# liyheng/MAGPO

Measured on NVIDIA B200. Metric: end_to_end_training_agent_env_steps_per_sec, higher is better.
Workload: dtype f32

## Files before the change

### magpo_b200/csrc/gemm_tc.cu

```cuda
#include <cuda.h>

#include <stdlib.h>

#include <vector>

#include "common.cuh"
#include "kernels.cuh"
#include "tc_ptx.cuh"

namespace magpo {
namespace {

using tcp::TC_BM;
constexpr int TC_KC = 32;
constexpr int TC_CHUNK_BYTES = TC_BM * TC_KC * 4;
constexpr int TC_CONV_THREADS = 256;
constexpr int TC_THREADS = 256 + TC_CONV_THREADS;
constexpr int TC_MAX_STAGES = 6;
constexpr uint32_t TC_SMEM_LIMIT = 227 * 1024;

struct TcParams {
  int M, N, K, BN, kchunks, stages, flags, num_row_tiles, tmem_cols, stacked ;
  const float* bias;
};
// ... 347 lines not shown
              CUtensorMapSwizzle swz = CU_TENSOR_MAP_SWIZZLE_128B) {
  EncodeTiledFn enc = get_encode();
  if (!enc) return false;
  cuuint64_t gdim[2] = {(cuuint64_t)cols, (cuuint64_t)rows};
  cuuint64_t gstride[1] = {(cuuint64_t)ld * 4};
  cuuint32_t box[2] = {(cuuint32_t)TC_KC, (cuuint32_t)box_rows};
  cuuint32_t estr[2] = {1, 1};
  return enc(tm, CU_TENSOR_MAP_DATA_TYPE_FLOAT32, 2, const_cast<float*>(ptr), gdim, gstride, box, estr, CU_TENSOR_MAP_INTERLEAVE_NONE,
             swz, CU_TENSOR_MAP_L2_PROMOTION_L2_128B, CU_TENSOR_MAP_FLOAT_OOB_FILL_NONE) == CUDA_SUCCESS;
}

bool env_tc_default() {
  const char* e = getenv("MAGPO_TENSOR_CORES");
  return !(e && e[0] == '0');
}
bool g_tc_enabled = env_tc_default();

}

bool tc_make_map(void* tensor_map, const float* ptr, int64_t rows, int cols, int ld, int box_rows) {
  return make_map(static_cast<CUtensorMap*>(tensor_map), ptr, rows, cols, ld, box_rows);
}
bool tc_make_map3(void* tensor_map, const float* ptr, int64_t T, int64_t rows, int cols, int box_rows) {
  EncodeTiledFn enc = get_encode();
  if (!enc) return false;
  cuuint64_t gdim[3] = {(cuuint64_t)cols, (cuuint64_t)rows, (cuuint64_t)T};
  cuuint64_t gstride[2] = {(cuuint64_t)cols * 4, (cuuint64_t)rows * cols * 4};
  cuuint32_t box[3] = {(cuuint32_t)TC_KC, (cuuint32_t)box_rows, 1};
  cuuint32_t estr[3] = {1, 1, 1};
  return enc(static_cast<CUtensorMap*>(tensor_map), CU_TENSOR_MAP_DATA_TYPE_FLOAT32, 3, const_cast<float*>(ptr), gdim, gstride, box, estr,
             CU_TENSOR_MAP_INTERLEAVE_NONE, CU_TENSOR_MAP_SWIZZLE_128B, CU_TENSOR_MAP_L2_PROMOTION_L2_128B,
             CU_TENSOR_MAP_FLOAT_OOB_FILL_NONE) == CUDA_SUCCESS;
}
void tc_set_enabled(bool on) { g_tc_enabled = on; }
bool tc_enabled() { return g_tc_enabled; }

int tc_prepare_region(cudaStream_t s, const float* base, int64_t n, float* hi, float* lo) {
  if (n <= 0) return MAGPO_OK;
  split_region_kernel<<<(unsigned)std::min<int64_t>(ceil_div(n, 256), 4 * kNumSMs), 256, 0, s>>>(n, base, hi, lo);
  MAGPO_LAUNCH_OK();
  auto overlaps = [](const float* a, int64_t na, const float* b, int64_t nb) { return a < b + nb && b < a + na; };
  std::vector<TcRegion>& g_regions = ctx().regions;
  for (size_t i = 0; i < g_regions.size();) {
    const TcRegion& r = g_regions[i];
    if (overlaps(r.base, r.n, base, n) || overlaps(r.base, r.n, hi, n) || overlaps(r.base, r.n, lo, n) ||
        overlaps(r.hi, r.n, base, n) || overlaps(r.lo, r.n, base, n))
      g_regions.erase(g_regions.begin() + (long)i);
    else
      ++i;
  }
  g_regions.push_back(TcRegion{base, n, hi, lo});
  return MAGPO_OK;
}

bool tc_lookup(const float* w, const float** hi, const float** lo) {
  const std::vector<TcRegion>& g_regions = ctx().regions;
  for (auto it = g_regions.rbegin(); it != g_regions.rend(); ++it) {
    const TcRegion& r = *it;
    if (w >= r.base && w < r.base + r.n) {
      *hi = r.hi + (w - r.base);
      *lo = r.lo + (w - r.base);
      return true;
    }
  }
  return false;
}
// ... 146 lines not shown
```

### magpo_b200/csrc/kernels.cuh

```cuda
#pragma once
#include "common.cuh"

namespace magpo {

constexpr int kD = 64;
constexpr int kH = 128;
constexpr int kMaxActions = 32;
constexpr int kMaxAgents = 8;

enum { GEMM_ACCUMULATE = 1, GEMM_RELU = 2 };

struct Wref {
  const float* w;
  int ldw;
  const float* wt;
  int ldwt;
};
inline Wref wref(const float* w, int ldw, const float* wt = nullptr, int ldwt = 0) { return Wref{w, ldw, wt, ldwt}; }

int gemm_nn(cudaStream_t s, int64_t M, int N, int K, const float* X, int ldx, Wref W, const float* bias, float* Y,
            int ldy, int flags);
void tc_set_enabled(bool on);
bool tc_enabled();
int tc_prepare_region(cudaStream_t s, const float* base, int64_t n, float* hi, float* lo);
bool tc_lookup(const float* w, const float** hi, const float** lo);
bool tc_supported(int64_t M, int N, int K, const float* X, int ldx, const float* Y, int ldy, int ldb);
int gemm_tc(cudaStream_t s, int64_t M, int N, int K, const float* X, int ldx, const float* Bhi, const float* Blo, int ldb,
            const float* bias, float* Y, int ldy, int flags);
bool tc_tn_supported(int64_t M, int N, int K, const float* X, int ldx, const float* dY, int ldy, const float* dW, int ldw);
int gemm_tc_tn(cudaStream_t s, int64_t M, int N, int K, const float* X, int ldx, const float* dY, int ldy, float* dW, int ldw);
bool tc_make_map(void* tensor_map, const float* ptr, int64_t rows, int cols, int ld, int box_rows);
bool tc_make_map3(void* tensor_map, const float* ptr, int64_t T, int64_t rows, int cols, int box_rows);
int gemm_tn(cudaStream_t s, int64_t M, int N, int K, const float* X, int ldx, const float* dY, int ldy, float* dW,
            int ldw);
void chain_set_enabled(bool on);
bool chain_supported(int64_t R);
int chain_gate_fwd(cudaStream_t s, int64_t R, const float* g, int ldg, const float* ret, const float* res, const float* gn_s,
                   const float* gn_b, const float* ln_s, const float* pe, const int32_t* step, int max_step, const float* W1T,
                   const float* W2T, const float* WpT, float* gated, float* o, float* y, float* ype, float* gl, float* hmid, float* proj,
                   int ldproj);
int chain_front_fwd(cudaStream_t s, int64_t R, int d, const float* obs, const float* obs_scale, const float* Wobs, int A, int a,
                    const int32_t* action, const float* Wa, const float* ln_s, const float* pe, const int32_t* step, int max_step,
                    const float* WqT, float* z0, float* x, float* xpe, float* qkvg);
int chain_tail_fwd(cudaStream_t s, int64_t R, const float* hmid, const float* res, const float* ln_s, const float* pe,
                   const int32_t* step, int max_step, const float* W1T, const float* WqT, int ldwq, const float* WhT, const float* h_bias,
                   const float* h2_s, const float* W3, const float* b3, int nout, float* f, float* x, float* xpe, float* q, int ldq,
                   float* zh, float* out);
int gru_scan_fwd(cudaStream_t s, int T, int N, int A, const float* gi, const float* WhT_hi, const float* WhT_lo, const float* bhn,
                 const uint8_t* done, float* rzn, float* ghn, float* Y, float* HU);
int gru_scan_bwd(cudaStream_t s, int T, int N, int A, const float* dY, const float* rzn, const float* ghn, const float* HU,
                 const uint8_t* done, const float* Wh_hi, const float* Wh_lo, float* dgi, float* dgh, float* dbi ,
                 float* dbhn );
int colsum(cudaStream_t s, int64_t M, int N, const float* dY, int ldy, float* db);
int transpose(cudaStream_t s, int R, int Cc, const float* in, float* out);

bool thin_k_ok(int K, int N, int ldw, const float* W, const float* Y, int ldy);
bool thin_n_ok(int K, int N, const float* X, int ldx);
bool obs_embed_ok(int d);
int thin_k_fwd(cudaStream_t s, int64_t R, int K, int N, const float* X, int ldx, const float* W, int ldw, const float* bias,
               float* Y, int ldy, int relu);
int thin_k_bwd(cudaStream_t s, int64_t R, int K, int N, const float* X, int ldx, const float* dY, int lddy, const float* relu_out,
               float* dW, int lddw, float* db);
int thin_n_fwd(cudaStream_t s, int64_t R, int K, int N, const float* X, int ldx, const float* W, int ldw, const float* bias,
               float* Y, int ldy);
int thin_n_bwd(cudaStream_t s, int64_t R, int K, int N, const float* X, int ldx, const float* dY, int lddy, const float* W, int ldw,
// ... 44 lines not shown
```

### magpo_b200/csrc/retention_chunk.cu

```cuda
#include "common.cuh"
#include "kernels.cuh"

namespace magpo {
namespace {

constexpr int RC_ROWS = 32;
constexpr int LDA = 68;
constexpr int LDB = 72;
constexpr int LDP = 36;
constexpr int LDPT = 40;

struct Frag {
  uint32_t h[4], l[4];
};
struct FragB {
  uint32_t h[2], l[2];
};

__device__ __forceinline__ void split(float x, uint32_t& hi, uint32_t& lo) {
  hi = __float_as_uint(x) & 0xFFFFE000u;
  lo = __float_as_uint(x - __uint_as_float(hi));
}

__device__ __forceinline__ void mma8(float (&c)[4], const uint32_t (&a)[4], const uint32_t (&b)[2]) {
  asm volatile(
      "mma.sync.aligned.m16n8k8.row.col.f32.tf32.tf32.f32 {%0,%1,%2,%3}, {%4,%5,%6,%7}, {%8,%9}, {%0,%1,%2,%3};"
      : "+f"(c[0]), "+f"(c[1]), "+f"(c[2]), "+f"(c[3])
      : "r"(a[0]), "r"(a[1]), "r"(a[2]), "r"(a[3]), "r"(b[0]), "r"(b[1]));
}
__device__ __forceinline__ void mma3(float (&c)[4], const Frag& a, const FragB& b) {
  mma8(c, a.l, b.h);
  mma8(c, a.h, b.l);
// ... 42 lines not shown
  ldsm_x2(Y + (n0 + (lane & 7)) * ld + k0 + ((lane >> 3) & 1) * 4, r);
  FragB f;
  split_u(r[0], f.h[0], f.l[0]);
  split_u(r[1], f.h[1], f.l[1]);
  return f;
}

__device__ __forceinline__ void zero4(float (&c)[4]) { c[0] = c[1] = c[2] = c[3] = 0.f; }

struct ChunkDecay {
  int cd_lane;
  __device__ __forceinline__ void init(const uint8_t* done, int t0, int L, int N, int n, int lane) {
    const bool d = done && lane < L && done[(int64_t)(t0 + lane) * N + n];
    const unsigned m = __ballot_sync(0xffffffffu, d);
    cd_lane = __popc(m & (0xffffffffu >> (31 - lane)));
  }
  __device__ __forceinline__ int cd(int tl) const { return __shfl_sync(0xffffffffu, cd_lane, tl); }
};

struct Tables {
  float* kpow;
  int* cds;
  uint8_t* row_tl;
};

template <bool CAUSAL>
__device__ __forceinline__ float decay_nm(const Tables& tb, int n, int m) {
  const int tn = tb.row_tl[n], tm = tb.row_tl[m];
  const bool order = CAUSAL ? (n >= m) : (tn >= tm);
  if (!order || tb.cds[tn] != tb.cds[tm]) return 0.f;
  return tb.kpow[tn - tm];
}

template <bool CAUSAL>
__global__ void __launch_bounds__(256, 2)
retention_chunk_fwd_kernel(int T, int N, int A, int Lc, float kappa, const float* __restrict__ q, const float* __restrict__ k,
                           const float* __restrict__ v, int ld, const float* __restrict__ H0, const uint8_t* __restrict__ done,
                           float* __restrict__ ret, float* __restrict__ Hck, float* __restrict__ Hout) {
  extern __shared__ __align__(16) float sm[];
  float* Hp = sm;
  float* Qs = Hp + 64 * LDB;
  float* Ks = Qs + RC_ROWS * LDA;
  float* Kt = Ks + RC_ROWS * LDA;
  float* Vs = Kt + RC_ROWS * LDB;
  float* Ps = Vs + RC_ROWS * LDB;
  Tables tb;
  tb.kpow = Ps + RC_ROWS * LDP;
  tb.cds = reinterpret_cast<int*>(tb.kpow + 40);
  tb.row_tl = reinterpret_cast<uint8_t*>(tb.cds + 32);

  const int n = blockIdx.x, tid = threadIdx.x, warp = tid >> 5, lane = tid & 31, g = lane >> 2, tq = lane & 3;
  if (tid == 0) {
    float p = 1.f;
    for (int j = 0; j < 40; ++j) { tb.kpow[j] = p; p *= kappa; }
  }
  if (tid < 32) tb.row_tl[tid] = (uint8_t)(tid / A);
  for (int i = tid; i < RC_ROWS * LDP; i += 256) Ps[i] = 0.f;

  const int mt = warp & 3, nt0 = (warp >> 2) * 4;
  float Hacc[4][4];
#pragma unroll
  for (int j = 0; j < 4; ++j) {
    const int r = 16 * mt + g, c = 8 * (nt0 + j) + 2 * tq;
    float2 lo2 = make_float2(0.f, 0.f), hi2 = make_float2(0.f, 0.f);
    if (H0) {
      lo2 = *reinterpret_cast<const float2*>(H0 + ((int64_t)n * 64 + r) * 64 + c);
      hi2 = *reinterpret_cast<const float2*>(H0 + ((int64_t)n * 64 + r + 8) * 64 + c);
    }
    Hacc[j][0] = lo2.x; Hacc[j][1] = lo2.y; Hacc[j][2] = hi2.x; Hacc[j][3] = hi2.y;
  }

  const int nchunks = (T + Lc - 1) / Lc;
  float pq[8], pk[8], pv[8];
  auto fetch = [&](int ch) {
    const int t0 = ch * Lc, L = min(Lc, T - t0), rows = L * A;
#pragma unroll
    for (int j = 0; j < 8; ++j) {
      const int idx = tid + j * 256, row = idx >> 6, col = idx & 63;
      pq[j] = pk[j] = pv[j] = 0.f;
      if (row < rows) {
        const int tl = tb.row_tl[row];
        const int64_t grow = ((int64_t)(t0 + tl) * N + n) * A + (row - tl * A);
        pq[j] = q[grow * ld + col]; pk[j] = k[grow * ld + col]; pv[j] = v[grow * ld + col];
      }
    }
  };
  __syncthreads();
  fetch(0);

  for (int ch = 0; ch < nchunks; ++ch) {
    const int t0 = ch * Lc, L = min(Lc, T - t0), rows = L * A;
    ChunkDecay cdk;
    cdk.init(done, t0, L, N, n, lane);
    const int cd_last = cdk.cd(L - 1);
    if (warp == 0) tb.cds[lane] = cdk.cd_lane;
#pragma unroll
    for (int j = 0; j < 4; ++j) {
      const int r = 16 * mt + g, c = 8 * (nt0 + j) + 2 * tq;
      *reinterpret_cast<float2*>(Hp + r * LDB + c) = make_float2(Hacc[j][0], Hacc[j][1]);
      *reinterpret_cast<float2*>(Hp + (r + 8) * LDB + c) = make_float2(Hacc[j][2], Hacc[j][3]);
      if (Hck) {
        float* dst = Hck + (((int64_t)ch * N + n) * 64) * 64;
        *reinterpret_cast<float2*>(dst + r * 64 + c) = make_float2(Hacc[j][0], Hacc[j][1]);
        *reinterpret_cast<float2*>(dst + (r + 8) * 64 + c) = make_float2(Hacc[j][2], Hacc[j][3]);
      }
    }
#pragma unroll
    for (int j = 0; j < 8; ++j) {
      const int idx = tid + j * 256, row = idx >> 6, col = idx & 63;
      const int tl = tb.row_tl[row];
      const int cdt = cdk.cd(tl);
      const float e = (row < rows && cdt == cd_last) ? tb.kpow[L - 1 - tl] : 0.f;
      Qs[row * LDA + col] = pq[j];
      Ks[row * LDA + col] = pk[j];
      Kt[row * LDB + col] = pk[j] * e;
      Vs[row * LDB + col] = pv[j];
    }
    __syncthreads();
    if (ch + 1 < nchunks) fetch(ch + 1);

    float o2[2][4];
    zero4(o2[0]); zero4(o2[1]);
    {
      const int mi = warp >> 2, ni = warp & 3;
      float s[4];
      zero4(s);
#pragma unroll
      for (int k0 = 0; k0 < 64; k0 += 8) {
        const Frag a0 = lda_row(Qs, LDA, 0, k0, g, tq);
        const Frag a1 = lda_row(Qs, LDA, 16, k0, g, tq);
        const FragB bk = ldb_tr(Ks, LDA, k0, 8 * ni, g, tq);
        mma3(s, mi ? a1 : a0, bk);
        const FragB bh = ldb(Hp, LDB, k0, 8 * warp, g, tq);
        mma3(o2[0], a0, bh);
        mma3(o2[1], a1, bh);
      }
      const int r = 16 * mi + g, c = 8 * ni + 2 * tq;
      Ps[r * LDP + c] = s[0] * decay_nm<CAUSAL>(tb, r, c);
      Ps[r * LDP + c + 1] = s[1] * decay_nm<CAUSAL>(tb, r, c + 1);
      Ps[(r + 8) * LDP + c] = s[2] * decay_nm<CAUSAL>(tb, r + 8, c);
      Ps[(r + 8) * LDP + c + 1] = s[3] * decay_nm<CAUSAL>(tb, r + 8, c + 1);
    }
    __syncthreads();

    {
      float o1[2][4];
      zero4(o1[0]); zero4(o1[1]);
#pragma unroll
      for (int k0 = 0; k0 < RC_ROWS; k0 += 8) {
        const FragB bv = ldb(Vs, LDB, k0, 8 * warp, g, tq);
        mma3(o1[0], lda_row(Ps, LDP, 0, k0, g, tq), bv);
        mma3(o1[1], lda_row(Ps, LDP, 16, k0, g, tq), bv);
      }
#pragma unroll
      for (int mi = 0; mi < 2; ++mi)
#pragma unroll
        for (int h = 0; h < 2; ++h) {
          const int row = 16 * mi + g + 8 * h;
          if (row < rows) {
            const int tl = tb.row_tl[row];
            const float cc = (tb.cds[tl] == 0) ? tb.kpow[tl + 1] : 0.f;
            const int64_t grow = ((int64_t)(t0 + tl) * N + n) * A + (row - tl * A);
            *reinterpret_cast<float2*>(ret + grow * 64 + 8 * warp + 2 * tq) =
                make_float2(o1[mi][2 * h] + cc * o2[mi][2 * h], o1[mi][2 * h + 1] + cc * o2[mi][2 * h + 1]);
          }
        }
    }
    {
      const float cL = (cd_last == 0) ? tb.kpow[L] : 0.f;
#pragma unroll
      for (int j = 0; j < 4; ++j)
#pragma unroll
        for (int x = 0; x < 4; ++x) Hacc[j][x] *= cL;
#pragma unroll
      for (int k0 = 0; k0 < RC_ROWS; k0 += 8) {
        const Frag a = lda_tr(Kt, LDB, 16 * mt, k0, g, tq);
#pragma unroll
        for (int j = 0; j < 4; ++j) mma3(Hacc[j], a, ldb(Vs, LDB, k0, 8 * (nt0 + j), g, tq));
      }
    }
    __syncthreads();
  }
  if (Hout) {
#pragma unroll
    for (int j = 0; j < 4; ++j) {
      const int r = 16 * mt + g, c = 8 * (nt0 + j) + 2 * tq;
      float* dst = Hout + (int64_t)n * 64 * 64;
      *reinterpret_cast<float2*>(dst + r * 64 + c) = make_float2(Hacc[j][0], Hacc[j][1]);
      *reinterpret_cast<float2*>(dst + (r + 8) * 64 + c) = make_float2(Hacc[j][2], Hacc[j][3]);
    }
  }
}

template <bool CAUSAL>
__global__ void __launch_bounds__(256, 2)
retention_chunk_bwd_kernel(int T, int N, int A, int Lc, float kappa, const float* __restrict__ q, const float* __restrict__ k,
                           const float* __restrict__ v, int ld, const uint8_t* __restrict__ done,
                           const float* __restrict__ Hck, const float* __restrict__ dret, float* __restrict__ dq,
                           float* __restrict__ dk, float* __restrict__ dv, int ldd) {
  extern __shared__ __align__(16) float sm[];
  float* Hp = sm;
  float* Gs = Hp + 64 * LDA;
  float* Gt = Gs + 64 * LDA;
  float* Qs = Gt + 64 * LDA;
  float* Ks = Qs + RC_ROWS * LDA;
  float* Vs = Ks + RC_ROWS * LDA;
  float* Ds = Vs + RC_ROWS * LDA;
  float* Qc = Ds + RC_ROWS * LDA;
  float* Ps = Qc + RC_ROWS * LDB;
  float* Ws = Ps + RC_ROWS * LDPT;
  Tables tb;
  tb.kpow = Ws + RC_ROWS * LDP;
  tb.cds = reinterpret_cast<int*>(tb.kpow + 40);
  tb.row_tl = reinterpret_cast<uint8_t*>(tb.cds + 32);

  const int n = blockIdx.x, tid = threadIdx.x, warp = tid >> 5, lane = tid & 31, g = lane >> 2, tq = lane & 3;
  if (tid == 0) {
    float p = 1.f;
    for (int j = 0; j < 40; ++j) { tb.kpow[j] = p; p *= kappa; }
  }
  if (tid < 32) tb.row_tl[tid] = (uint8_t)(tid / A);

  const int mt = warp & 3, nt0 = (warp >> 2) * 4;
// ... 130 lines not shown
          if (row < rows) {
            const int tl = tb.row_tl[row];
            const int cdt = tb.cds[tl];
            const float cc = (cdt == 0) ? tb.kpow[tl + 1] : 0.f;
            const float ee = (cdt == cd_last) ? tb.kpow[L - 1 - tl] : 0.f;
            const int64_t grow = ((int64_t)(t0 + tl) * N + n) * A + (row - tl * A);
            const int col = 8 * warp + 2 * tq;
            *reinterpret_cast<float2*>(dq + grow * ldd + col) =
                make_float2(dq1[mi][2 * h] + cc * dq2[mi][2 * h], dq1[mi][2 * h + 1] + cc * dq2[mi][2 * h + 1]);
            *reinterpret_cast<float2*>(dk + grow * ldd + col) =
                make_float2(dk1[mi][2 * h] + ee * dk2[mi][2 * h], dk1[mi][2 * h + 1] + ee * dk2[mi][2 * h + 1]);
            *reinterpret_cast<float2*>(dv + grow * ldd + col) =
                make_float2(dv1[mi][2 * h] + ee * dv2[mi][2 * h], dv1[mi][2 * h + 1] + ee * dv2[mi][2 * h + 1]);
          }
        }
    }
    {
      const float cL = (cd_last == 0) ? tb.kpow[L] : 0.f;
#pragma unroll
      for (int j = 0; j < 4; ++j)
#pragma unroll
        for (int x = 0; x < 4; ++x) Gacc[j][x] *= cL;
#pragma unroll
      for (int k0 = 0; k0 < RC_ROWS; k0 += 8) {
        const Frag a = lda_tr(Qc, LDB, 16 * mt, k0, g, tq);
#pragma unroll
        for (int j = 0; j < 4; ++j) mma3(Gacc[j], a, ldb(Ds, LDA, k0, 8 * (nt0 + j), g, tq));
      }
    }
    __syncthreads();
  }
}

constexpr size_t kFwdSmem = (size_t)(64 * LDB + 2 * RC_ROWS * LDA + 2 * RC_ROWS * LDB + RC_ROWS * LDP + 40 + 32 + 8) * sizeof(float);
constexpr size_t kBwdSmem =
    (size_t)(3 * 64 * LDA + 4 * RC_ROWS * LDA + RC_ROWS * LDB + RC_ROWS * LDPT + RC_ROWS * LDP + 40 + 32 + 8) * sizeof(float);

template <typename Kern>
int set_smem(Kern kern, size_t bytes) {
  MAGPO_CUDA_OK(cudaFuncSetAttribute(kern, cudaFuncAttributeMaxDynamicSharedMemorySize, (int)bytes));
  return MAGPO_OK;
}

}

int retention_chunk_len(int A) { return std::max(1, RC_ROWS / A); }
int retention_num_chunks(int T, int A) { return (T + retention_chunk_len(A) - 1) / retention_chunk_len(A); }

int retention_chunk_fwd(cudaStream_t s, int T, int N, int A, float kappa, bool causal, const float* q, const float* k,
                        const float* v, int ld, const float* H0, const uint8_t* done, float* ret, float* Hck, float* Hout) {
  const int Lc = retention_chunk_len(A);
  if (once_per_device(ONCE_RET_FWD)) {
    MAGPO_TRY(set_smem(retention_chunk_fwd_kernel<true>, kFwdSmem));
    MAGPO_TRY(set_smem(retention_chunk_fwd_kernel<false>, kFwdSmem));
  }
  ProfScope ps(PROF_RET_FWD, s, 4.0 * 256.0 * (double)T * N * A);
  if (causal)
    retention_chunk_fwd_kernel<true><<<N, 256, kFwdSmem, s>>>(T, N, A, Lc, kappa, q, k, v, ld, H0, done, ret, Hck, Hout);
  else
    retention_chunk_fwd_kernel<false><<<N, 256, kFwdSmem, s>>>(T, N, A, Lc, kappa, q, k, v, ld, H0, done, ret, Hck, Hout);
  MAGPO_LAUNCH_OK();
  return MAGPO_OK;
}

int retention_chunk_bwd(cudaStream_t s, int T, int N, int A, float kappa, bool causal, const float* q, const float* k,
                        const float* v, int ld, const uint8_t* done, const float* Hck, const float* dret, float* dq,
                        float* dk, float* dv, int ldd) {
  const int Lc = retention_chunk_len(A);
  if (once_per_device(ONCE_RET_BWD)) {
    MAGPO_TRY(set_smem(retention_chunk_bwd_kernel<true>, kBwdSmem));
    MAGPO_TRY(set_smem(retention_chunk_bwd_kernel<false>, kBwdSmem));
  }
  ProfScope ps(PROF_RET_BWD, s, 7.0 * 256.0 * (double)T * N * A);
  if (causal)
    retention_chunk_bwd_kernel<true><<<N, 256, kBwdSmem, s>>>(T, N, A, Lc, kappa, q, k, v, ld, done, Hck, dret, dq, dk, dv, ldd);
  else
    retention_chunk_bwd_kernel<false><<<N, 256, kBwdSmem, s>>>(T, N, A, Lc, kappa, q, k, v, ld, done, Hck, dret, dq, dk, dv, ldd);
  MAGPO_LAUNCH_OK();
  return MAGPO_OK;
}

}
```

### magpo_b200/csrc/tc_ptx.cuh

```cuda
#pragma once
#include <cuda.h>
#include <stdint.h>

namespace magpo {
namespace tcp {

constexpr int TC_BM = 128;
__device__ __forceinline__ uint32_t smem_u32(const void* p) { return (uint32_t)__cvta_generic_to_shared(p); }
__device__ __forceinline__ void mbar_init(uint64_t* bar, uint32_t count) {
  asm volatile("mbarrier.init.shared::cta.b64 [%0], %1;" ::"r"(smem_u32(bar)), "r"(count) : "memory");
}
__device__ __forceinline__ void mbar_expect_tx(uint64_t* bar, uint32_t bytes) {
  asm volatile("mbarrier.arrive.expect_tx.shared::cta.b64 _, [%0], %1;" ::"r"(smem_u32(bar)), "r"(bytes) : "memory");
}
__device__ __forceinline__ void mbar_arrive(uint64_t* bar) {
  asm volatile("mbarrier.arrive.shared::cta.b64 _, [%0];" ::"r"(smem_u32(bar)) : "memory");
}
__device__ __forceinline__ bool mbar_try_wait(uint64_t* bar, uint32_t parity) {
  uint32_t ok;
  asm volatile(
      "{\n\t.reg .pred P1;\n\tmbarrier.try_wait.parity.shared::cta.b64 P1, [%1], %2;\n\tselp.b32 %0, 1, 0, P1;\n\t}"
      : "=r"(ok)
      : "r"(smem_u32(bar)), "r"(parity)
      : "memory");
  return ok != 0;
}
__device__ __forceinline__ void mbar_wait(uint64_t* bar, uint32_t parity) {
  for (uint32_t spins = 0; !mbar_try_wait(bar, parity); ++spins)
    if (spins > (1u << 24)) __trap();
}
__device__ __forceinline__ void tma_load_2d(void* dst, const CUtensorMap* tm, int c0, int c1, uint64_t* bar) {
  asm volatile(
      "cp.async.bulk.tensor.2d.shared::cluster.global.mbarrier::complete_tx::bytes [%0], [%1, {%3, %4}], [%2];" ::"r"(
          smem_u32(dst)),
      "l"(reinterpret_cast<uint64_t>(tm)), "r"(smem_u32(bar)), "r"(c0), "r"(c1)
      : "memory");
}
__device__ __forceinline__ void tma_load_3d(void* dst, const CUtensorMap* tm, int c0, int c1, int c2, uint64_t* bar) {
  asm volatile(
      "cp.async.bulk.tensor.3d.shared::cluster.global.mbarrier::complete_tx::bytes [%0], [%1, {%3, %4, %5}], [%2];" ::"r"(
          smem_u32(dst)),
      "l"(reinterpret_cast<uint64_t>(tm)), "r"(smem_u32(bar)), "r"(c0), "r"(c1), "r"(c2)
      : "memory");
}
__device__ __forceinline__ void tma_store_2d(const CUtensorMap* tm, const void* src, int c0, int c1) {
  asm volatile("cp.async.bulk.tensor.2d.global.shared::cta.bulk_group [%0, {%2, %3}], [%1];" ::"l"(
                   reinterpret_cast<uint64_t>(tm)),
               "r"(smem_u32(src)), "r"(c0), "r"(c1)
               : "memory");
}
__device__ __forceinline__ void tma_store_3d(const CUtensorMap* tm, const void* src, int c0, int c1, int c2) {
  asm volatile("cp.async.bulk.tensor.3d.global.shared::cta.bulk_group [%0, {%2, %3, %4}], [%1];" ::"l"(reinterpret_cast<uint64_t>(tm)),
               "r"(smem_u32(src)), "r"(c0), "r"(c1), "r"(c2)
               : "memory");
}
__device__ __forceinline__ void tma_reduce_add_2d(const CUtensorMap* tm, const void* src, int c0, int c1) {
  asm volatile("cp.reduce.async.bulk.tensor.2d.global.shared::cta.add.bulk_group [%0, {%2, %3}], [%1];" ::"l"(
                   reinterpret_cast<uint64_t>(tm)),
               "r"(smem_u32(src)), "r"(c0), "r"(c1)
               : "memory");
}
__device__ __forceinline__ void bulk_commit() { asm volatile("cp.async.bulk.commit_group;" ::: "memory"); }
template <int N>
__device__ __forceinline__ void bulk_wait_read() {
  asm volatile("cp.async.bulk.wait_group.read %0;" ::"n"(N) : "memory");
}
__device__ __forceinline__ void bulk_wait_all() { asm volatile("cp.async.bulk.wait_group 0;" ::: "memory"); }
__device__ __forceinline__ void fence_proxy_async() { asm volatile("fence.proxy.async.shared::cta;" ::: "memory"); }
__device__ __forceinline__ void fence_barrier_init() { asm volatile("fence.mbarrier_init.release.cluster;" ::: "memory"); }
__device__ __forceinline__ void tc_fence_before() { asm volatile("tcgen05.fence::before_thread_sync;" ::: "memory"); }
__device__ __forceinline__ void tc_fence_after() { asm volatile("tcgen05.fence::after_thread_sync;" ::: "memory"); }
__device__ __forceinline__ void umma_commit(uint64_t* bar) {
  asm volatile("tcgen05.commit.cta_group::1.mbarrier::arrive::one.shared::cluster.b64 [%0];" ::"r"(smem_u32(bar)) : "memory");
}
__device__ __forceinline__ void umma_tf32(uint32_t tmem_d, uint64_t adesc, uint64_t bdesc, uint32_t idesc, uint32_t accumulate) {
// ... 49 lines not shown
```

Measured before the change: 8.446 million.

## Rewrite retention chunk forward on tcgen05 UMMA with TMA loads and persistent grid

Replaces the mma.sync-based retention chunk forward kernel with a 128-thread persistent kernel. It loads q/k/v chunks through 4D TMA tensor maps with mbarriers, prefetching the next chunk, and computes QK^T and the P·V plus Q·H terms with 3-pass split-TF32 tcgen05 MMAs accumulating in tensor memory. The recurrent state H is held in registers of two warps, and the grid is capped at twice the SM count. This adds tensor-memory allocation, synchronisation and split-precision overhead, and assumes rows per chunk fit within 32 and a feature width of 64.

Result: slower. 8.069 million (median of 6 runs) (-4.5%).

```diff
diff --git a/magpo_b200/csrc/gemm_tc.cu b/magpo_b200/csrc/gemm_tc.cu
--- a/magpo_b200/csrc/gemm_tc.cu
+++ b/magpo_b200/csrc/gemm_tc.cu
@@ -403,6 +403,17 @@
              CU_TENSOR_MAP_INTERLEAVE_NONE, CU_TENSOR_MAP_SWIZZLE_128B, CU_TENSOR_MAP_L2_PROMOTION_L2_128B,
              CU_TENSOR_MAP_FLOAT_OOB_FILL_NONE) == CUDA_SUCCESS;
 }
+bool tc_make_map_env_rows(void* tensor_map, const float* ptr, int T, int N, int A, int ld, int Lc) {
+  EncodeTiledFn enc = get_encode();
+  if (!enc) return false;
+  cuuint64_t gdim[4] = {64, (cuuint64_t)A, (cuuint64_t)N, (cuuint64_t)T};
+  cuuint64_t gstride[3] = {(cuuint64_t)ld * 4, (cuuint64_t)A * ld * 4, (cuuint64_t)N * A * ld * 4};
+  cuuint32_t box[4] = {(cuuint32_t)TC_KC, (cuuint32_t)A, 1, (cuuint32_t)Lc};
+  cuuint32_t estr[4] = {1, 1, 1, 1};
+  return enc(static_cast<CUtensorMap*>(tensor_map), CU_TENSOR_MAP_DATA_TYPE_FLOAT32, 4, const_cast<float*>(ptr), gdim, gstride, box, estr,
+             CU_TENSOR_MAP_INTERLEAVE_NONE, CU_TENSOR_MAP_SWIZZLE_128B, CU_TENSOR_MAP_L2_PROMOTION_L2_128B,
+             CU_TENSOR_MAP_FLOAT_OOB_FILL_NONE) == CUDA_SUCCESS;
+}
 void tc_set_enabled(bool on) { g_tc_enabled = on; }
 bool tc_enabled() { return g_tc_enabled; }
 
diff --git a/magpo_b200/csrc/kernels.cuh b/magpo_b200/csrc/kernels.cuh
--- a/magpo_b200/csrc/kernels.cuh
+++ b/magpo_b200/csrc/kernels.cuh
@@ -31,6 +31,7 @@
 int gemm_tc_tn(cudaStream_t s, int64_t M, int N, int K, const float* X, int ldx, const float* dY, int ldy, float* dW, int ldw);
 bool tc_make_map(void* tensor_map, const float* ptr, int64_t rows, int cols, int ld, int box_rows);
 bool tc_make_map3(void* tensor_map, const float* ptr, int64_t T, int64_t rows, int cols, int box_rows);
+bool tc_make_map_env_rows(void* tensor_map, const float* ptr, int T, int N, int A, int ld, int Lc);
 int gemm_tn(cudaStream_t s, int64_t M, int N, int K, const float* X, int ldx, const float* dY, int ldy, float* dW,
             int ldw);
 void chain_set_enabled(bool on);
diff --git a/magpo_b200/csrc/retention_chunk.cu b/magpo_b200/csrc/retention_chunk.cu
--- a/magpo_b200/csrc/retention_chunk.cu
+++ b/magpo_b200/csrc/retention_chunk.cu
@@ -1,3 +1,4 @@
+#include "chain.cuh"
 #include "common.cuh"
 #include "kernels.cuh"
 
@@ -106,163 +107,306 @@
   return tb.kpow[tn - tm];
 }
 
+constexpr int RF_THREADS = 128;
+constexpr uint32_t RF_TM_COLS = 256;
+constexpr int RF_TM_ALO = 96, RF_TM_D = 192;
+constexpr int RF_QRAW = 0;
+constexpr int RF_KRAW = 8192;
+constexpr int RF_VRAW = 16384;
+constexpr int RF_QLO = 24576;
+constexpr int RF_KLO = 32768;
+constexpr int RF_VTH = 40960;
+constexpr int RF_VTL = 49152;
+constexpr int RF_HTH = 57344;
+constexpr int RF_HTL = 73728;
+constexpr int RF_TAB = 90112;
+constexpr size_t kFwdSmem = 1024 + RF_TAB + 1024;
+static_assert(RF_QLO + 4096 + 128 * 128 <= RF_TAB, "MMA1 A rows stay inside shared memory");
+
+__device__ __forceinline__ int sw128(int row, int col) { return row * 128 + ((((col >> 2) ^ row) & 7) << 4) + ((col & 3) << 2); }
+__device__ __forceinline__ void row_read32(const uint8_t* blk, int row, float (&x)[32]) {
+  const float4* src = reinterpret_cast<const float4*>(blk + row * 128);
+#pragma unroll
+  for (int j = 0; j < 8; ++j) {
+    const float4 t = src[j ^ (row & 7)];
+    x[4 * j] = t.x; x[4 * j + 1] = t.y; x[4 * j + 2] = t.z; x[4 * j + 3] = t.w;
+  }
+}
+__device__ __forceinline__ void row_write32(uint8_t* blk, int row, const float (&x)[32]) {
+  float4* dst = reinterpret_cast<float4*>(blk + row * 128);
+#pragma unroll
+  for (int j = 0; j < 8; ++j) dst[j ^ (row & 7)] = make_float4(x[4 * j], x[4 * j + 1], x[4 * j + 2], x[4 * j + 3]);
+}
+__device__ __forceinline__ void tmem_st16(uint32_t taddr, const uint32_t* v) {
+  asm volatile(
+      "tcgen05.st.sync.aligned.32x32b.x16.b32 [%0], {%1, %2, %3, %4, %5, %6, %7, %8, %9, %10, %11, %12, %13, %14, %15, %16};" ::"r"(taddr),
+      "r"(v[0]), "r"(v[1]), "r"(v[2]), "r"(v[3]), "r"(v[4]), "r"(v[5]), "r"(v[6]), "r"(v[7]), "r"(v[8]), "r"(v[9]), "r"(v[10]),
+      "r"(v[11]), "r"(v[12]), "r"(v[13]), "r"(v[14]), "r"(v[15])
+      : "memory");
+}
+__device__ __forceinline__ void tmem_put_split(uint32_t taddr_hi, uint32_t taddr_lo, const float (&x)[32]) {
+#pragma unroll
+  for (int h = 0; h < 2; ++h) {
+    uint32_t hi[16], lo[16];
+#pragma unroll
+    for (int j = 0; j < 16; ++j) split(x[16 * h + j], hi[j], lo[j]);
+    tmem_st16(taddr_hi + 16 * h, hi);
+    tmem_st16(taddr_lo + 16 * h, lo);
+  }
+}
+
 template <bool CAUSAL>
-__global__ void __launch_bounds__(256, 2)
-retention_chunk_fwd_kernel(int T, int N, int A, int Lc, float kappa, const float* __restrict__ q, const float* __restrict__ k,
-                           const float* __restrict__ v, int ld, const float* __restrict__ H0, const uint8_t* __restrict__ done,
-                           float* __restrict__ ret, float* __restrict__ Hck, float* __restrict__ Hout) {
-  extern __shared__ __align__(16) float sm[];
-  float* Hp = sm;
-  float* Qs = Hp + 64 * LDB;
-  float* Ks = Qs + RC_ROWS * LDA;
-  float* Kt = Ks + RC_ROWS * LDA;
-  float* Vs = Kt + RC_ROWS * LDB;
-  float* Ps = Vs + RC_ROWS * LDB;
-  Tables tb;
-  tb.kpow = Ps + RC_ROWS * LDP;
-  tb.cds = reinterpret_cast<int*>(tb.kpow + 40);
-  tb.row_tl = reinterpret_cast<uint8_t*>(tb.cds + 32);
-
-  const int n = blockIdx.x, tid = threadIdx.x, warp = tid >> 5, lane = tid & 31, g = lane >> 2, tq = lane & 3;
+__global__ void __launch_bounds__(RF_THREADS, 2)
+retention_chunk_fwd_kernel(const __grid_constant__ CUtensorMap tmq, const __grid_constant__ CUtensorMap tmk,
+                           const __grid_constant__ CUtensorMap tmv, int T, int N, int A, int Lc, float kappa,
+                           const float* __restrict__ H0, const uint8_t* __restrict__ done, float* __restrict__ ret,
+                           float* __restrict__ Hck, float* __restrict__ Hout) {
+  using namespace tcp;
+  extern __shared__ uint8_t rf_smem_raw[];
+  uint8_t* sm = reinterpret_cast<uint8_t*>((reinterpret_cast<uintptr_t>(rf_smem_raw) + 1023) & ~uintptr_t(1023));
+  float* kpow = reinterpret_cast<float*>(sm + RF_TAB);
+  int* cdw = reinterpret_cast<int*>(sm + RF_TAB + 160);
+  uint8_t* row_tl = sm + RF_TAB + 672;
+  uint64_t* bars = reinterpret_cast<uint64_t*>(sm + RF_TAB + 704);
+  uint32_t* tmem_ptr = reinterpret_cast<uint32_t*>(bars + 3);
+
+  const int tid = threadIdx.x, warp = tid >> 5, lane = tid & 31;
   if (tid == 0) {
     float p = 1.f;
-    for (int j = 0; j < 40; ++j) { tb.kpow[j] = p; p *= kappa; }
-  }
-  if (tid < 32) tb.row_tl[tid] = (uint8_t)(tid / A);
-  for (int i = tid; i < RC_ROWS * LDP; i += 256) Ps[i] = 0.f;
-
-  const int mt = warp & 3, nt0 = (warp >> 2) * 4;
-  float Hacc[4][4];
-#pragma unroll
-  for (int j = 0; j < 4; ++j) {
-    const int r = 16 * mt + g, c = 8 * (nt0 + j) + 2 * tq;
-    float2 lo2 = make_float2(0.f, 0.f), hi2 = make_float2(0.f, 0.f);
-    if (H0) {
-      lo2 = *reinterpret_cast<const float2*>(H0 + ((int64_t)n * 64 + r) * 64 + c);
-      hi2 = *reinterpret_cast<const float2*>(H0 + ((int64_t)n * 64 + r + 8) * 64 + c);
-    }
-    Hacc[j][0] = lo2.x; Hacc[j][1] = lo2.y; Hacc[j][2] = hi2.x; Hacc[j][3] = hi2.y;
+    for (int j = 0; j < 40; ++j) { kpow[j] = p; p *= kappa; }
+    for (int i = 0; i < 3; ++i) mbar_init(&bars[i], 1);
+    fence_barrier_init();
+  }
+  if (tid < 32) row_tl[tid] = (uint8_t)(tid / A);
+  if (warp == 0) {
+    asm volatile("tcgen05.alloc.cta_group::1.sync.aligned.shared::cta.b32 [%0], %1;" ::"r"(smem_u32(tmem_ptr)), "r"(RF_TM_COLS) : "memory");
+    asm volatile("tcgen05.relinquish_alloc_permit.cta_group::1.sync.aligned;" ::: "memory");
+  }
+  tc_fence_before();
+  __syncthreads();
+  tc_fence_after();
+  const uint32_t tmem = *tmem_ptr;
+  const uint32_t tm_lane = tmem + ((uint32_t)(warp * 32) << 16);
+  if (warp >= 2) {
+    uint32_t z[32];
+#pragma unroll
+    for (int j = 0; j < 32; ++j) z[j] = 0u;
+    chain::tmem_st32(tm_lane + 32, z);
+    chain::tmem_st32(tm_lane + 64, z);
+    chain::tmem_st32(tm_lane + RF_TM_ALO + 32, z);
+    chain::tmem_st32(tm_lane + RF_TM_ALO + 64, z);
+    chain::tmem_st_wait();
   }
 
   const int nchunks = (T + Lc - 1) / Lc;
-  float pq[8], pk[8], pv[8];
-  auto fetch = [&](int ch) {
-    const int t0 = ch * Lc, L = min(Lc, T - t0), rows = L * A;
-#pragma unroll
-    for (int j = 0; j < 8; ++j) {
-      const int idx = tid + j * 256, row = idx >> 6, col = idx & 63;
-      pq[j] = pk[j] = pv[j] = 0.f;
-      if (row < rows) {
-        const int tl = tb.row_tl[row];
-        const int64_t grow = ((int64_t)(t0 + tl) * N + n) * A + (row - tl * A);
-        pq[j] = q[grow * ld + col]; pk[j] = k[grow * ld + col]; pv[j] = v[grow * ld + col];
-      }
+  const uint32_t tx_bytes = 3u * 2u * 128u * (uint32_t)(Lc * A);
+  auto load_chunk = [&](int n, int ch) {
+    mbar_expect_tx(&bars[0], tx_bytes);
+#pragma unroll
+    for (int b = 0; b < 2; ++b) {
+      tma_load_4d(sm + RF_QRAW + 4096 * b, &tmq, 32 * b, 0, n, ch * Lc, &bars[0]);
+      tma_load_4d(sm + RF_KRAW + 4096 * b, &tmk, 32 * b, 0, n, ch * Lc, &bars[0]);
+      tma_load_4d(sm + RF_VRAW + 4096 * b, &tmv, 32 * b, 0, n, ch * Lc, &bars[0]);
     }
   };
+  auto load_done = [&](int n, int ch) {
+    const int t = ch * Lc + lane;
+    return done && lane < Lc && t < T && done[(int64_t)t * N + n] != 0;
+  };
+  if (tid == 0) load_chunk(blockIdx.x, 0);
+  bool d_next = load_done(blockIdx.x, 0);
+
+  uint32_t it = 0;
+  float H[64];
+  for (int n = blockIdx.x; n < N; n += gridDim.x) {
+    if (warp >= 2) {
+      const int r = tid - 64;
+#pragma unroll
+      for (int j = 0; j < 16; ++j) {
+        const float4 h = H0 ? reinterpret_cast<const float4*>(H0 + ((int64_t)n * 64 + r) * 64)[j] : make_float4(0.f, 0.f, 0.f, 0.f);
+        H[4 * j] = h.x; H[4 * j + 1] = h.y; H[4 * j + 2] = h.z; H[4 * j + 3] = h.w;
+      }
+    }
+    for (int ch = 0; ch < nchunks; ++ch, ++it) {
+      const int t0 = ch * Lc, L = min(Lc, T - t0), rows = L * A;
+      const uint32_t ph = it & 1u;
+      int* cd = cdw + 32 * warp;
+      {
+        const unsigned m = __ballot_sync(0xffffffffu, d_next);
+        cd[lane] = __popc(m & (0xffffffffu >> (31 - lane)));
+        __syncwarp();
+        if (ch + 1 < nchunks) d_next = load_done(n, ch + 1);
+        else if (n + (int)gridDim.x < N) d_next = load_done(n + gridDim.x, 0);
+      }
+      const int cd_last = cd[L - 1];
+
+      if (warp >= 2) {
+        const int r = tid - 64;
+        uint8_t* hth = sm + RF_HTH + 8192 * (r >> 5);
+        uint8_t* htl = sm + RF_HTL + 8192 * (r >> 5);
+#pragma unroll
+        for (int c = 0; c < 64; ++c) {
+          const int off = sw128(c, r & 31);
+          *reinterpret_cast<float*>(hth + off) = H[c];
+          *reinterpret_cast<float*>(htl + off) = tf32_residual(H[c]);
+        }
+        if (Hck) {
+          float4* dst = reinterpret_cast<float4*>(Hck + (((int64_t)ch * N + n) * 64 + r) * 64);
+#pragma unroll
+          for (int j = 0; j < 16; ++j) dst[j] = make_float4(H[4 * j], H[4 * j + 1], H[4 * j + 2], H[4 * j + 3]);
+        }
+      }
+      mbar_wait(&bars[0], ph);
+      if (warp == 0) {
+        const int row = lane, tl = row_tl[row];
+        const float cc = (row < rows && cd[tl] == 0) ? kpow[tl + 1] : 0.f;
+#pragma unroll
+        for (int b = 0; b < 2; ++b) {
+          float x[32];
+          row_read32(sm + RF_QRAW + 4096 * b, row, x);
+#pragma unroll
+          for (int j = 0; j < 32; ++j) x[j] *= cc;
+          tmem_put_split(tm_lane + 32 + 32 * b, tm_lane + RF_TM_ALO + 32 + 32 * b, x);
+          row_read32(sm + RF_QRAW + 4096 * b, row, x);
+#pragma unroll
+          for (int j = 0; j < 32; ++j) x[j] = tf32_residual(x[j]);
+          row_write32(sm + RF_QLO + 4096 * b, row, x);
+        }
+      } else if (warp == 1) {
+        const int m = lane;
+        const bool valid = m < rows;
+#pragma unroll
+        for (int b = 0; b < 2; ++b) {
+          float x[32];
+          row_read32(sm + RF_KRAW + 4096 * b, m, x);
+#pragma unroll
+          for (int j = 0; j < 32; ++j) x[j] = tf32_residual(x[j]);
+          row_write32(sm + RF_KLO + 4096 * b, m, x);
+          row_read32(sm + RF_VRAW + 4096 * b, m, x);
+#pragma unroll
+          for (int j = 0; j < 32; ++j) {
+            const int off = sw128(32 * b + j, m);
+            const float v = valid ? x[j] : 0.f;
+            *reinterpret_cast<float*>(sm + RF_VTH + off) = v;
+            *reinterpret_cast<float*>(sm + RF_VTL + off) = tf32_residual(v);
+          }
+        }
+      } else {
+        const int r = tid - 64;
+        const uint8_t* kb = sm + RF_KRAW + 4096 * (r >> 5);
+        float x[32];
+#pragma unroll
+        for (int m = 0; m < 32; ++m) {
+          const int tm = row_tl[m];
+          const bool ok = m < rows && cd[tm] == cd_last;
+          const float kv = *reinterpret_cast<const float*>(kb + sw128(m, r & 31));
+          x[m] = ok ? kpow[max(L - 1 - tm, 0)] * kv : 0.f;
+        }
+        tmem_put_split(tm_lane, tm_lane + RF_TM_ALO, x);
+      }
+      chain::tmem_st_wait();
+      fence_proxy_async();
+      tc_fence_before();
+      __syncthreads();
+
+      if (tid == 0) {
+        tc_fence_after();
+        const uint32_t idesc = umma_idesc_tf32(32);
+        const uint32_t qh = smem_u32(sm + RF_QRAW), ql = smem_u32(sm + RF_QLO), kh = smem_u32(sm + RF_KRAW), kl = smem_u32(sm + RF_KLO);
+#pragma unroll
+        for (int kk = 0; kk < 8; ++kk) {
+          const uint32_t o = 4096u * (kk >> 2) + 32u * (kk & 3);
+          umma_tf32(tmem + RF_TM_D, umma_desc_k_sw128(ql + o), umma_desc_k_sw128(kh + o), idesc, kk ? 1u : 0u);
+          umma_tf32(tmem + RF_TM_D, umma_desc_k_sw128(qh + o), umma_desc_k_sw128(kl + o), idesc, 1u);
+          umma_tf32(tmem + RF_TM_D, umma_desc_k_sw128(qh + o), umma_desc_k_sw128(kh + o), idesc, 1u);
+        }
+        umma_commit(&bars[1]);
+      }
+      __syncwarp();
+      if (warp == 0) {
+        mbar_wait(&bars[1], ph);
+        __syncwarp();
+        tc_fence_after();
+        if (lane == 0) {
+          if (ch + 1 < nchunks) load_chunk(n, ch + 1);
+          else if (n + (int)gridDim.x < N) load_chunk(n + gridDim.x, 0);
+        }
+        uint32_t s[32];
+        tmem_ld32(tm_lane + RF_TM_D, s);
+        const int row = lane, tn = row_tl[row], cdn = cd[tn];
+        float x[32];
+#pragma unroll
+        for (int m = 0; m < 32; ++m) {
+          const int tm = row_tl[m];
+          const bool ok = m < rows && (CAUSAL ? row >= m : tn >= tm) && cdn == cd[tm];
+          x[m] = ok ? kpow[max(tn - tm, 0)] * __uint_as_float(s[m]) : 0.f;
+        }
+        tmem_put_split(tm_lane, tm_lane + RF_TM_ALO, x);
+        chain::tmem_st_wait();
+      }
+      tc_fence_before();
+      __syncthreads();
+
+      if (tid == 0) {
+        tc_fence_after();
+        const uint32_t idesc = umma_idesc_tf32(64);
+        const uint32_t vh = smem_u32(sm + RF_VTH), vl = smem_u32(sm + RF_VTL), hh = smem_u32(sm + RF_HTH), hl = smem_u32(sm + RF_HTL);
+#pragma unroll
+        for (int kk = 0; kk < 12; ++kk) {
+          const uint32_t bh = kk < 4 ? vh + 32u * kk : hh + 8192u * ((kk - 4) >> 2) + 32u * ((kk - 4) & 3);
+          const uint32_t bl = kk < 4 ? vl + 32u * kk : hl + 8192u * ((kk - 4) >> 2) + 32u * ((kk - 4) & 3);
+          const uint32_t a = tmem + 8u * kk;
+          chain::umma_tf32_ts(tmem + RF_TM_D, a + RF_TM_ALO, umma_desc_k_sw128(bh), idesc, kk ? 1u : 0u);
+          chain::umma_tf32_ts(tmem + RF_TM_D, a, umma_desc_k_sw128(bl), idesc, 1u);
+          chain::umma_tf32_ts(tmem + RF_TM_D, a, umma_desc_k_sw128(bh), idesc, 1u);
+        }
+        umma_commit(&bars[2]);
+      }
+      __syncwarp();
+      mbar_wait(&bars[2], ph);
+      __syncwarp();
+      tc_fence_after();
+      if (warp == 0) {
+        uint32_t o0[32], o1[32];
+        chain::tmem_ld32_nowait(tm_lane + RF_TM_D, o0);
+        chain::tmem_ld32_nowait(tm_lane + RF_TM_D + 32, o1);
+        chain::tmem_ld_wait();
+        const int row = lane;
+        if (row < rows) {
+          const int tl = row_tl[row];
+          float4* dst = reinterpret_cast<float4*>(ret + (((int64_t)(t0 + tl) * N + n) * A + (row - tl * A)) * 64);
+#pragma unroll
+          for (int j = 0; j < 8; ++j) {
+            dst[j] = make_float4(__uint_as_float(o0[4 * j]), __uint_as_float(o0[4 * j + 1]), __uint_as_float(o0[4 * j + 2]),
+                                 __uint_as_float(o0[4 * j + 3]));
+            dst[8 + j] = make_float4(__uint_as_float(o1[4 * j]), __uint_as_float(o1[4 * j + 1]), __uint_as_float(o1[4 * j + 2]),
+                                     __uint_as_float(o1[4 * j + 3]));
+          }
+        }
+      } else if (warp >= 2) {
+        const float cL = (cd_last == 0) ? kpow[L] : 0.f;
+#pragma unroll
+        for (int h = 0; h < 2; ++h) {
+          uint32_t d[32];
+          tmem_ld32(tm_lane + RF_TM_D + 32 * h, d);
+#pragma unroll
+          for (int j = 0; j < 32; ++j) H[32 * h + j] = cL * H[32 * h + j] + __uint_as_float(d[j]);
+        }
+      }
+      tc_fence_before();
+      __syncwarp();
+    }
+    if (warp >= 2 && Hout) {
+      float4* dst = reinterpret_cast<float4*>(Hout + ((int64_t)n * 64 + (tid - 64)) * 64);
+#pragma unroll
+      for (int j = 0; j < 16; ++j) dst[j] = make_float4(H[4 * j], H[4 * j + 1], H[4 * j + 2], H[4 * j + 3]);
+    }
+  }
+  tc_fence_before();
   __syncthreads();
-  fetch(0);
-
-  for (int ch = 0; ch < nchunks; ++ch) {
-    const int t0 = ch * Lc, L = min(Lc, T - t0), rows = L * A;
-    ChunkDecay cdk;
-    cdk.init(done, t0, L, N, n, lane);
-    const int cd_last = cdk.cd(L - 1);
-    if (warp == 0) tb.cds[lane] = cdk.cd_lane;
-#pragma unroll
-    for (int j = 0; j < 4; ++j) {
-      const int r = 16 * mt + g, c = 8 * (nt0 + j) + 2 * tq;
-      *reinterpret_cast<float2*>(Hp + r * LDB + c) = make_float2(Hacc[j][0], Hacc[j][1]);
-      *reinterpret_cast<float2*>(Hp + (r + 8) * LDB + c) = make_float2(Hacc[j][2], Hacc[j][3]);
-      if (Hck) {
-        float* dst = Hck + (((int64_t)ch * N + n) * 64) * 64;
-        *reinterpret_cast<float2*>(dst + r * 64 + c) = make_float2(Hacc[j][0], Hacc[j][1]);
-        *reinterpret_cast<float2*>(dst + (r + 8) * 64 + c) = make_float2(Hacc[j][2], Hacc[j][3]);
-      }
-    }
-#pragma unroll
-    for (int j = 0; j < 8; ++j) {
-      const int idx = tid + j * 256, row = idx >> 6, col = idx & 63;
-      const int tl = tb.row_tl[row];
-      const int cdt = cdk.cd(tl);
-      const float e = (row < rows && cdt == cd_last) ? tb.kpow[L - 1 - tl] : 0.f;
-      Qs[row * LDA + col] = pq[j];
-      Ks[row * LDA + col] = pk[j];
-      Kt[row * LDB + col] = pk[j] * e;
-      Vs[row * LDB + col] = pv[j];
-    }
-    __syncthreads();
-    if (ch + 1 < nchunks) fetch(ch + 1);
-
-    float o2[2][4];
-    zero4(o2[0]); zero4(o2[1]);
-    {
-      const int mi = warp >> 2, ni = warp & 3;
-      float s[4];
-      zero4(s);
-#pragma unroll
-      for (int k0 = 0; k0 < 64; k0 += 8) {
-        const Frag a0 = lda_row(Qs, LDA, 0, k0, g, tq);
-        const Frag a1 = lda_row(Qs, LDA, 16, k0, g, tq);
-        const FragB bk = ldb_tr(Ks, LDA, k0, 8 * ni, g, tq);
-        mma3(s, mi ? a1 : a0, bk);
-        const FragB bh = ldb(Hp, LDB, k0, 8 * warp, g, tq);
-        mma3(o2[0], a0, bh);
-        mma3(o2[1], a1, bh);
-      }
-      const int r = 16 * mi + g, c = 8 * ni + 2 * tq;
-      Ps[r * LDP + c] = s[0] * decay_nm<CAUSAL>(tb, r, c);
-      Ps[r * LDP + c + 1] = s[1] * decay_nm<CAUSAL>(tb, r, c + 1);
-      Ps[(r + 8) * LDP + c] = s[2] * decay_nm<CAUSAL>(tb, r + 8, c);
-      Ps[(r + 8) * LDP + c + 1] = s[3] * decay_nm<CAUSAL>(tb, r + 8, c + 1);
-    }
-    __syncthreads();
-
-    {
-      float o1[2][4];
-      zero4(o1[0]); zero4(o1[1]);
-#pragma unroll
-      for (int k0 = 0; k0 < RC_ROWS; k0 += 8) {
-        const FragB bv = ldb(Vs, LDB, k0, 8 * warp, g, tq);
-        mma3(o1[0], lda_row(Ps, LDP, 0, k0, g, tq), bv);
-        mma3(o1[1], lda_row(Ps, LDP, 16, k0, g, tq), bv);
-      }
-#pragma unroll
-      for (int mi = 0; mi < 2; ++mi)
-#pragma unroll
-        for (int h = 0; h < 2; ++h) {
-          const int row = 16 * mi + g + 8 * h;
-          if (row < rows) {
-            const int tl = tb.row_tl[row];
-            const float cc = (tb.cds[tl] == 0) ? tb.kpow[tl + 1] : 0.f;
-            const int64_t grow = ((int64_t)(t0 + tl) * N + n) * A + (row - tl * A);
-            *reinterpret_cast<float2*>(ret + grow * 64 + 8 * warp + 2 * tq) =
-                make_float2(o1[mi][2 * h] + cc * o2[mi][2 * h], o1[mi][2 * h + 1] + cc * o2[mi][2 * h + 1]);
-          }
-        }
-    }
-    {
-      const float cL = (cd_last == 0) ? tb.kpow[L] : 0.f;
-#pragma unroll
-      for (int j = 0; j < 4; ++j)
-#pragma unroll
-        for (int x = 0; x < 4; ++x) Hacc[j][x] *= cL;
-#pragma unroll
-      for (int k0 = 0; k0 < RC_ROWS; k0 += 8) {
-        const Frag a = lda_tr(Kt, LDB, 16 * mt, k0, g, tq);
-#pragma unroll
-        for (int j = 0; j < 4; ++j) mma3(Hacc[j], a, ldb(Vs, LDB, k0, 8 * (nt0 + j), g, tq));
-      }
-    }
-    __syncthreads();
-  }
-  if (Hout) {
-#pragma unroll
-    for (int j = 0; j < 4; ++j) {
-      const int r = 16 * mt + g, c = 8 * (nt0 + j) + 2 * tq;
-      float* dst = Hout + (int64_t)n * 64 * 64;
-      *reinterpret_cast<float2*>(dst + r * 64 + c) = make_float2(Hacc[j][0], Hacc[j][1]);
-      *reinterpret_cast<float2*>(dst + (r + 8) * 64 + c) = make_float2(Hacc[j][2], Hacc[j][3]);
-    }
+  if (warp == 0) {
+    tc_fence_after();
+    asm volatile("tcgen05.dealloc.cta_group::1.sync.aligned.b32 %0, %1;" ::"r"(tmem), "r"(RF_TM_COLS) : "memory");
   }
 }
 
@@ -459,7 +603,6 @@
   }
 }
 
-constexpr size_t kFwdSmem = (size_t)(64 * LDB + 2 * RC_ROWS * LDA + 2 * RC_ROWS * LDB + RC_ROWS * LDP + 40 + 32 + 8) * sizeof(float);
 constexpr size_t kBwdSmem =
     (size_t)(3 * 64 * LDA + 4 * RC_ROWS * LDA + RC_ROWS * LDB + RC_ROWS * LDPT + RC_ROWS * LDP + 40 + 32 + 8) * sizeof(float);
 
@@ -477,15 +620,20 @@
 int retention_chunk_fwd(cudaStream_t s, int T, int N, int A, float kappa, bool causal, const float* q, const float* k,
                         const float* v, int ld, const float* H0, const uint8_t* done, float* ret, float* Hck, float* Hout) {
   const int Lc = retention_chunk_len(A);
+  CUtensorMap mq, mk, mv;
+  if (!tc_make_map_env_rows(&mq, q, T, N, A, ld, Lc) || !tc_make_map_env_rows(&mk, k, T, N, A, ld, Lc) ||
+      !tc_make_map_env_rows(&mv, v, T, N, A, ld, Lc))
+    return MAGPO_ERR_UNSUPPORTED;
   if (once_per_device(ONCE_RET_FWD)) {
     MAGPO_TRY(set_smem(retention_chunk_fwd_kernel<true>, kFwdSmem));
     MAGPO_TRY(set_smem(retention_chunk_fwd_kernel<false>, kFwdSmem));
   }
   ProfScope ps(PROF_RET_FWD, s, 4.0 * 256.0 * (double)T * N * A);
+  const int grid = std::min(N, 2 * kNumSMs);
   if (causal)
-    retention_chunk_fwd_kernel<true><<<N, 256, kFwdSmem, s>>>(T, N, A, Lc, kappa, q, k, v, ld, H0, done, ret, Hck, Hout);
+    retention_chunk_fwd_kernel<true><<<grid, RF_THREADS, kFwdSmem, s>>>(mq, mk, mv, T, N, A, Lc, kappa, H0, done, ret, Hck, Hout);
   else
-    retention_chunk_fwd_kernel<false><<<N, 256, kFwdSmem, s>>>(T, N, A, Lc, kappa, q, k, v, ld, H0, done, ret, Hck, Hout);
+    retention_chunk_fwd_kernel<false><<<grid, RF_THREADS, kFwdSmem, s>>>(mq, mk, mv, T, N, A, Lc, kappa, H0, done, ret, Hck, Hout);
   MAGPO_LAUNCH_OK();
   return MAGPO_OK;
 }
diff --git a/magpo_b200/csrc/tc_ptx.cuh b/magpo_b200/csrc/tc_ptx.cuh
--- a/magpo_b200/csrc/tc_ptx.cuh
+++ b/magpo_b200/csrc/tc_ptx.cuh
@@ -41,6 +41,13 @@
       "cp.async.bulk.tensor.3d.shared::cluster.global.mbarrier::complete_tx::bytes [%0], [%1, {%3, %4, %5}], [%2];" ::"r"(
           smem_u32(dst)),
       "l"(reinterpret_cast<uint64_t>(tm)), "r"(smem_u32(bar)), "r"(c0), "r"(c1), "r"(c2)
+      : "memory");
+}
+__device__ __forceinline__ void tma_load_4d(void* dst, const CUtensorMap* tm, int c0, int c1, int c2, int c3, uint64_t* bar) {
+  asm volatile(
+      "cp.async.bulk.tensor.4d.shared::cluster.global.mbarrier::complete_tx::bytes [%0], [%1, {%3, %4, %5, %6}], [%2];" ::"r"(
+          smem_u32(dst)),
+      "l"(reinterpret_cast<uint64_t>(tm)), "r"(smem_u32(bar)), "r"(c0), "r"(c1), "r"(c2), "r"(c3)
       : "memory");
 }
 __device__ __forceinline__ void tma_store_2d(const CUtensorMap* tm, const void* src, int c0, int c1) {
```
